# RustCrypto/elliptic-curves

Measured on AMD Instinct MI355X. Metric: k256 fixed-base scalar-muls/sec (variable-time: mul_by_generator_vartime), higher is better.
Workload: dtype u32 limbs (v_mad_u64_u32); 1 GPU; fixed_k256; curve=k256, units_per_gpu=1048576, units_total=1048576, window_bits=default, parallelism=shard1, input_sets=4, form=variable-time comb (ecgpu_batch_mul_base_dev = mul_by_generator_vartime)

## Files before the change

elliptic-curves_amd/csrc/ecgpu_batchinv.h:

```cpp
#pragma once

#include "ecgpu_point.h"
#include "ecgpu_scalar.h"

namespace ecgpu {

template <class R, class Load, class More, class Work>
ECGPU_HD void chain_walk(size_t first, size_t step, Load load, More has_next, Work work) {
    R cur, next;
    bool more = true;
    for (size_t j = first, it = 0;; j += step, it++) {
        if (more) load(j, next);
        if (it) work(j - step, cur);
        if (!more) break;
        cur = next;
        more = has_next(j);
    }
}

template <class P>
ECGPU_HD void batch_inv_lane(size_t t, size_t n, size_t nthreads, P& p) {
    using El = typename P::El;
    using Fwd = typename P::Fwd;
    using Back = typename P::Back;
    if (t >= n) return;
    El acc = p.one();
    chain_walk<Fwd>(t, nthreads, [&](size_t j, Fwd& r) { p.load_fwd(j, r); }, [&](size_t j) { return j + nthreads < n; },
                    [&](size_t j, const Fwd& r) {
                        El f;
                        const uint32_t cls = p.classify(j, r, f);
                        p.put_prefix(j, acc, cls);
                        if (cls == 0) acc = p.mul(acc, f);
                    });
    El inv = p.inv(acc);
    chain_walk<Back>(t + (n - 1 - t) / nthreads * nthreads, (size_t)0 - nthreads, [&](size_t j, Back& r) { p.load_back(j, r); },
                     [&](size_t j) { return j >= nthreads; },
                     [&](size_t j, const Back& r) {
                         El f, own;
                         const uint32_t cls = p.classify(j, r, f);
                         if (cls == 0) {
                             own = p.mul(p.prefix(j, r), inv);
                             inv = p.mul(inv, f);
                         }
                         p.emit(j, r, cls, own);
                     });
}

template <class Rec>
struct FieldLane : Rec {
    using F = typename Rec::F;
    using El = typename Rec::El;
    static constexpr int NL = Rec::NL, NS = Rec::NS;
    static_assert(NS > NL, "raw form has no spare word");
    ECGPU_HD El one() const { return F::one(); }
    ECGPU_HD El mul(const El& a, const El& b) const { return F::mul(a, b); }
    ECGPU_HD El inv(const El& a) const { return F::inv(a); }
    ECGPU_HD void put_prefix(size_t j, const El& acc, uint32_t cls) const {
        uint32_t w[NS];
#pragma unroll
        for (int i = 0; i < NS; i++) w[i] = i < NL ? acc.e.v[i] : 0u;
        w[NS - 1] = cls;
        this->io.put_prefix(j, w);
    }
    ECGPU_HD El prefix(size_t, const typename Rec::Back& r) const {
        Fe<NL> e;
#pragma unroll
        for (int i = 0; i < NL; i++) e.v[i] = r.pw[i];
        return F::template wrap<1, 1>(e);
    }
};

enum : int { NORM_WIRE = 0, NORM_PACKED = 1, NORM_COMPRESSED = 2 };
template <class C, int MODE, class Io>
struct NormRec {
    using F = Field<C>;
    using G = Group<C>;
    using El = typename F::M1;
    static constexpr int N = C::N, NL = C::NL, NS = F::NS;
    struct Fwd { Fe<NL> z; };
    struct Back { Proj<C> p; uint32_t pw[NS]; };
    Io& io;
    ECGPU_HD void load_fwd(size_t j, Fwd& r) const { r.z = io.load_z(j); }
    ECGPU_HD void load_back(size_t j, Back& r) const { r.p = io.load_point(j); io.get_prefix(j, r.pw); }
    ECGPU_HD uint32_t classify(size_t, const Fwd& r, El& f) const {
        f = G::m(r.z);
        return F::is_zero(f) ? 1u : 0u;
    }
    ECGPU_HD uint32_t classify(size_t, const Back& r, El& f) const {
        f = G::m(r.p.z);
        return r.pw[NS - 1];
    }
    ECGPU_HD void coord(uint32_t* w, const El& v) const {
        if constexpr (MODE == NORM_PACKED) F::pack(w, v);
        else F::to_canonical(w, v);
    }
    ECGPU_HD void emit(size_t j, const Back& r, uint32_t cls, const El& zinv) const {
        uint32_t w[N];
        if (cls) {
            if (MODE == NORM_PACKED) return;
#pragma unroll
            for (int i = 0; i < N; i++) w[i] = 0u;
            io.put_x(j, w);
            if (MODE == NORM_WIRE) io.put_y(j, w);
            io.put_flag(j, MODE == NORM_WIRE ? 1 : 0);
            return;
        }
        const El x = F::mul(G::m(r.p.x), zinv), y = F::mul(G::m(r.p.y), zinv);
        coord(w, x);
        io.put_x(j, w);
        coord(w, y);
        if (MODE != NORM_COMPRESSED) io.put_y(j, w);
        if (MODE != NORM_PACKED) io.put_flag(j, MODE == NORM_WIRE ? 0 : (uint8_t)(2u + (w[0] & 1u)));
    }
};
template <class C, int MODE, class Io>
ECGPU_HD void normalize_lane(size_t t, size_t n, size_t nthreads, Io& io) {
    FieldLane<NormRec<C, MODE, Io>> lane{{io}};
    batch_inv_lane(t, n, nthreads, lane);
}

template <class C, class Io>
struct ScalarInvLane {
    using S = ScalarN<C>;
    static constexpr int N = C::N;
    struct El { uint32_t v[N]; };
    struct Fwd {};
    struct Back {};
    Io& io;
    ECGPU_HD El one() const {
        El r = {{1u}};
        S::to_mont(r.v, r.v);
        return r;
    }
    ECGPU_HD El mul(const El& a, const El& b) const {
        El r;
        S::mont_mul(r.v, a.v, b.v);
        return r;
    }
    ECGPU_HD El inv(const El& acc) const {
        El x;
        S::inv(x.v, acc.v);
        S::to_mont(x.v, x.v);
        S::to_mont(x.v, x.v);
        return x;
    }
    ECGPU_HD void load_fwd(size_t, Fwd&) const {}
    ECGPU_HD void load_back(size_t, Back&) const {}
    template <class R>
    ECGPU_HD uint32_t classify(size_t j, const R&, El& f) const {
        uint32_t a[N];
        io.load(j, a);
        if (S::is_zero(a) || !S::in_range(a)) return 1u;
        S::to_mont(f.v, a);
        return 0u;
    }
    ECGPU_HD void put_prefix(size_t j, const El& acc, uint32_t) const { io.put_prefix(j, acc.v); }
    ECGPU_HD El prefix(size_t j, const Back&) const {
        El e;
        io.get_prefix(j, e.v);
        return e;
    }
    ECGPU_HD void emit(size_t j, const Back&, uint32_t cls, const El& ainv) const {
        El w = {};
        if (!cls) S::from_mont(w.v, ainv.v);
        io.put(j, w.v);
    }
};
template <class C, class Io>
ECGPU_HD void scalar_batch_inv_lane(size_t t, size_t n, size_t nthreads, Io& io) {
    ScalarInvLane<C, Io> lane{io};
    batch_inv_lane(t, n, nthreads, lane);
}

}
```

elliptic-curves_amd/csrc/ecgpu_field.h:

```cpp
#pragma once

#include "ecgpu_params.h"
#include "ecgpu_modinv.h"
#ifndef ECGPU_K256_ASM_REDUCE
#define ECGPU_K256_ASM_REDUCE 1
#endif
#if ECGPU_K256_ASM_REDUCE && defined(__HIP_DEVICE_COMPILE__) && (defined(__gfx950__) || defined(__gfx942__))
#define ECGPU_K256_ASM_REDUCE_ON 1
#include "ecgpu_k256_reduce_asm.h"
#else
#define ECGPU_K256_ASM_REDUCE_ON 0
#endif

namespace ecgpu {

template <class C, int L, int V>
struct Mag {
    Fe<C::NL> e;
};

static ECGPU_HD uint32_t opaque_const(uint32_t x) {
#if defined(__HIP_DEVICE_COMPILE__)
    asm("" : "+s"(x));
#endif
    return x;
}

template <class C>
struct Field {
    ECGPU_CONST int N = C::N;
    ECGPU_CONST int NL = C::NL;
    ECGPU_CONST int NS = (C::NL / 4 + 1) * 4;
    ECGPU_CONST int REPR = C::REPR;
    using E = Fe<C::NL>;
    using M1 = Mag<C, 1, 1>;

    ECGPU_CONST int MAXPROD = REPR == REPR_U29_K256 ? 7 : C::UC::MAXPROD;
    ECGPU_CONST int MAXMAG = REPR == REPR_U29_K256 ? 7 : C::UC::MAXMAG;

    using KC = consts::K256U;
    ECGPU_CONST uint32_t KMASK = (1u << 29) - 1;

    static ECGPU_HD void k_fold(uint64_t* lo, int j, uint64_t col) {
        uint32_t cl = (uint32_t)col, ch = (uint32_t)(col >> 32);
        lo[j] += (uint64_t)cl * KC::F0;
        lo[j + 1] += (uint64_t)cl * opaque_const(KC::F1);
        lo[j + 1] += (uint64_t)ch * KC::G1;
        lo[j + 2] += (uint64_t)ch * opaque_const(KC::G2);
    }
    static ECGPU_HD E k_reduce(uint64_t* c) {
#if ECGPU_K256_ASM_REDUCE_ON
        if constexpr (REPR == REPR_U29_K256) return k256_reduce_asm(c, KC::F0, KC::F1, KC::G1, KC::G2);
#endif
        return k_reduce_cpp(c);
    }
    static ECGPU_HD E k_reduce_cpp(uint64_t* c) {
        uint64_t lo[11];
#pragma unroll
        for (int k = 0; k < 9; k++) lo[k] = c[k];
        lo[9] = 0;
        lo[10] = 0;
#pragma unroll
        for (int k = 9; k < 16; k++) {
            const uint32_t cl = (uint32_t)c[k], ch = (uint32_t)(c[k] >> 32);
            c[k + 1] += (uint64_t)ch * opaque_const(8u);
            lo[k - 9] += (uint64_t)cl * KC::F0;
            lo[k - 8] += (uint64_t)cl * opaque_const(KC::F1);
        }
        k_fold(lo, 7, c[16]);
        {
            uint64_t c9 = lo[9], c10 = lo[10];
            const uint32_t cl = (uint32_t)c9, ch = (uint32_t)(c9 >> 32);
            c10 += (uint64_t)ch * opaque_const(8u);
            lo[0] += (uint64_t)cl * KC::F0;
            lo[1] += (uint64_t)cl * opaque_const(KC::F1);
            k_fold(lo, 1, c10);
        }
        E r;
        uint64_t v = lo[0];
#pragma unroll
        for (int k = 0; k < 8; k++) {
            r.v[k] = (uint32_t)v & KMASK;
            v = lo[k + 1] + (v >> 29);
        }
        r.v[8] = (uint32_t)v & KMASK;
        uint64_t top = v >> 29;
        uint32_t tl = (uint32_t)top, th = (uint32_t)(top >> 32);
        uint64_t t0 = (uint64_t)tl * KC::F0 + r.v[0];
        uint64_t t1 = (uint64_t)tl * opaque_const(KC::F1) + r.v[1];
        t1 += (uint64_t)th * KC::G1;
        uint64_t t2 = (uint64_t)th * opaque_const(KC::G2) + r.v[2];
        r.v[0] = (uint32_t)t0 & KMASK;
        t1 += t0 >> 29;
        r.v[1] = (uint32_t)t1 & KMASK;
        t2 += t1 >> 29;
        r.v[2] = (uint32_t)t2 & KMASK;
        r.v[3] += (uint32_t)(t2 >> 29);
        return r;
    }
    static ECGPU_HD void k_columns(uint64_t* c, const uint32_t* a, const uint32_t* b, bool accumulate) {
        if (!accumulate) {
#pragma unroll
            for (int k = 0; k < 17; k++) c[k] = 0;
        }
#pragma unroll
        for (int i = 0; i < 9; i++) {
#pragma unroll
            for (int j = 0; j < 9; j++) c[i + j] += (uint64_t)a[i] * b[j];
        }
    }
    static ECGPU_HD void k_columns_sqr(uint64_t* c, const uint32_t* a) {
        uint32_t a2[9];
#pragma unroll
        for (int k = 0; k < 17; k++) c[k] = 0;
#pragma unroll
        for (int j = 0; j < 9; j++) a2[j] = a[j] << 1;
#pragma unroll
        for (int i = 0; i < 9; i++) {
            c[2 * i] += (uint64_t)a[i] * a[i];
#pragma unroll
            for (int j = i + 1; j < 9; j++) c[i + j] += (uint64_t)a[i] * a2[j];
        }
    }
    static ECGPU_HD E k_norm(const E& a) {
        E r;
        uint32_t carry = 0;
#pragma unroll
        for (int k = 0; k < 9; k++) {
            uint32_t v = a.v[k] + carry;
            r.v[k] = v & KMASK;
            carry = v >> 29;
        }
        r.v[0] += carry * KC::F0;
        r.v[1] += carry * KC::F1;
        return r;
    }
    static ECGPU_HD E k_mul_small(const E& a, uint32_t k) {
        E r;
        uint64_t t = 0;
#pragma unroll
        for (int i = 0; i < 9; i++) {
            t += (uint64_t)a.v[i] * k;
            r.v[i] = (uint32_t)t & KMASK;
            t >>= 29;
        }
        uint32_t top = (uint32_t)t;
        uint64_t t0 = (uint64_t)top * KC::F0 + r.v[0];
        uint64_t t1 = (uint64_t)top * KC::F1 + r.v[1] + (t0 >> 29);
        r.v[0] = (uint32_t)t0 & KMASK;
        r.v[1] = (uint32_t)t1 & KMASK;
        r.v[2] += (uint32_t)(t1 >> 29);
        return r;
    }
    template <bool NORMED = false>
    static ECGPU_HD void k_to_words(uint32_t* w, const E& a) {
        E r;
        if constexpr (NORMED) r = a;
        else r = k_norm(k_norm(a));
#pragma unroll
        for (int rep = 0; rep < 2; rep++) {
            uint32_t carry = 0;
#pragma unroll
            for (int k = 0; k < 8; k++) {
                uint32_t v = r.v[k] + carry;
                r.v[k] = v & KMASK;
                carry = v >> 29;
            }
            uint32_t v8 = r.v[8] + carry;
            uint32_t e = v8 >> 24;
            r.v[8] = v8 & 0xFFFFFFu;
            r.v[0] += e * 977u;
            r.v[1] += e * 8u;
        }
        {
            uint32_t carry = 0;
#pragma unroll
            for (int k = 0; k < 8; k++) {
                uint32_t v = r.v[k] + carry;
                r.v[k] = v & KMASK;
                carry = v >> 29;
            }
            r.v[8] += carry;
        }
        E s = r;
        s.v[0] += 977u;
        s.v[1] += 8u;
        {
            uint32_t carry = 0;
#pragma unroll
            for (int k = 0; k < 8; k++) {
                uint32_t v = s.v[k] + carry;
                s.v[k] = v & KMASK;
                carry = v >> 29;
            }
            s.v[8] += carry;
        }
        bool ge = (s.v[8] >> 24) != 0;
        s.v[8] &= 0xFFFFFFu;
#pragma unroll
        for (int k = 0; k < 9; k++) r.v[k] = ge ? s.v[k] : r.v[k];
#pragma unroll
        for (int i = 0; i < 8; i++) {
            int bit = 32 * i, l = bit / 29, sh = bit % 29;
            uint64_t x = (uint64_t)r.v[l] >> sh;
            x |= (uint64_t)r.v[l + 1] << (29 - sh);
            if (l + 2 < 9) x |= (uint64_t)r.v[l + 2] << (58 - sh);
            w[i] = (uint32_t)x;
        }
    }
    template <int NLIMB, int BITS>
    static ECGPU_HD E words_to_limbs(const uint32_t* w) {
        E r;
#pragma unroll
        for (int l = 0; l < NLIMB; l++) {
            int bit = BITS * l, i = bit / 32, sh = bit % 32;
            uint64_t x = i < N ? (uint64_t)w[i] >> sh : 0;
            if (i + 1 < N) x |= (uint64_t)w[i + 1] << (32 - sh);
            r.v[l] = (uint32_t)x & ((1u << BITS) - 1);
        }
        return r;
    }

    using PC = typename C::UC;
    ECGPU_CONST int UN = PC::NL, UB = PC::B;
    ECGPU_CONST uint32_t PMASK = (1u << PC::B) - 1;

    static ECGPU_HD E p_reduce(uint64_t* c) {
        if constexpr (C::ID == CURVE_P256) {
#pragma unroll
            for (int i = 0; i < UN; i++) {
                uint32_t u = (uint32_t)c[i] & PMASK;
                c[i + 1] += (c[i] >> UB);
                c[i + 3] += (uint64_t)u * opaque_const(1u << 12);
                c[i + 6] += (uint64_t)u * opaque_const(1u << 24);
                c[i + 8] += (uint64_t)u * opaque_const(0xFFFFFFFFu);
            }
            E r;
            uint64_t v = c[UN];
#pragma unroll
            for (int k = 0; k < UN - 1; k++) {
                r.v[k] = (uint32_t)v & PMASK;
                v = c[UN + 1 + k] + (v >> UB);
            }
            r.v[UN - 1] = (uint32_t)v;
            return r;
        }
        if constexpr (C::ID == CURVE_P384) {
#pragma unroll
            for (int i = 0; i < UN; i++) {
                const int64_t ci = (int64_t)c[i];
                const int64_t u = (int64_t)((uint32_t)ci & PMASK);
                c[i + 1] = (uint64_t)((int64_t)c[i + 1] + (ci >> UB) + u * (int64_t)(int32_t)opaque_const(1u << 5));
                c[i + 3] = (uint64_t)((int64_t)c[i + 3] + u * (int64_t)(int32_t)opaque_const(0u - (1u << 15)));
                c[i + 4] = (uint64_t)((int64_t)c[i + 4] + u * (int64_t)(int32_t)opaque_const(0u - (1u << 20)));
                c[i + 14] = (uint64_t)((int64_t)c[i + 14] + u * (int64_t)(int32_t)opaque_const(1u << 6));
            }
            E r;
            int64_t v = (int64_t)c[UN];
#pragma unroll
            for (int k = 0; k < UN - 1; k++) {
                r.v[k] = (uint32_t)v & PMASK;
                v = (int64_t)c[UN + 1 + k] + (v >> UB);
            }
            r.v[UN - 1] = (uint32_t)v;
            return r;
        }
        if constexpr (C::ID == CURVE_P521) {
#pragma unroll
            for (int i = 0; i < UN; i++) {
                uint32_t u = (uint32_t)c[i] & PMASK;
                c[i + 1] += (c[i] >> UB);
                c[i + 19] += (uint64_t)u << 8;
            }
            E r;
            uint64_t v = c[UN];
#pragma unroll
            for (int k = 0; k < UN - 1; k++) {
                r.v[k] = (uint32_t)v & PMASK;
                v = c[UN + 1 + k] + (v >> UB);
            }
            r.v[UN - 1] = (uint32_t)v;
            return r;
        }
        if constexpr (C::ID == CURVE_SM2 || C::ID == CURVE_P224 || C::ID == CURVE_P192) {
            static_assert(HasBias<PC>::value, "sparse rows need the column biases");
#pragma unroll
            for (int i = 0; i < UN; i++) {
                uint32_t u;
                if constexpr (C::ID == CURVE_P224) {
                    u = (0u - (uint32_t)c[i]) & PMASK;
                    c[i + 1] += (c[i] + u) >> UB;
                } else {
                    u = (uint32_t)c[i] & PMASK;
                    c[i + 1] += c[i] >> UB;
                }
                const int64_t su = (int64_t)u;
                if constexpr (C::ID == CURVE_SM2) {
                    c[i + 2] += (uint64_t)u * opaque_const(1u << 8);
                    c[i + 3] = (uint64_t)((int64_t)c[i + 3] + su * (int64_t)(int32_t)opaque_const(0u - (1u << 12)));
                    c[i + 8] += (uint64_t)u * opaque_const(0xFFFFFFFFu);
                } else if constexpr (C::ID == CURVE_P224) {
                    c[i + 3] = (uint64_t)((int64_t)c[i + 3] + su * (int64_t)(int32_t)opaque_const(0u - (1u << 15)));
                    c[i + 8] += (uint64_t)u * opaque_const(1u << 8);
                } else {
                    c[i + 2] = (uint64_t)((int64_t)c[i + 2] + su * (int64_t)(int32_t)opaque_const(0u - (1u << 12)));
                    c[i + 7] += (uint64_t)u * opaque_const(1u << 10);
                }
            }
            E r;
            uint64_t v = c[UN];
#pragma unroll
            for (int k = 0; k < UN - 1; k++) {
                r.v[k] = (uint32_t)v & PMASK;
                v = c[UN + 1 + k] + (v >> UB);
            }
            r.v[UN - 1] = (uint32_t)v;
            return r;
        }
        if constexpr (C::ID == CURVE_BIGN256) {
            static_assert(UB == 28 && UN == 10, "bign256: 10 x 28 limbs");
#pragma unroll
            for (int i = 0; i < UN; i++) {
                const int64_t ci = (int64_t)c[i];
                const int64_t u = (int64_t)(((uint32_t)ci * PC::PINV) & PMASK);
                const int64_t t = ci + u * (int64_t)(int32_t)opaque_const(0u - 189u);
                c[i + 1] = (uint64_t)((int64_t)c[i + 1] + (t >> UB));
                c[i + 9] = (uint64_t)((int64_t)c[i + 9] + u * (int64_t)(int32_t)opaque_const(16u));
            }
            E r;
            int64_t v = (int64_t)c[UN];
#pragma unroll
            for (int k = 0; k < UN - 1; k++) {
                r.v[k] = (uint32_t)v & PMASK;
                v = (int64_t)c[UN + 1 + k] + (v >> UB);
            }
            r.v[UN - 1] = (uint32_t)v;
            return r;
        }
        if constexpr (!PC::P0_IS_MINUS_ONE && !PC::P0_IS_ONE) {
#pragma unroll
            for (int i = 0; i < UN; i++) {
                uint32_t u = ((uint32_t)c[i] * PC::PINV) & PMASK;
#pragma unroll
                for (int j = 0; j < UN; j++) {
                    if (PC::P[j] != 0) c[i + j] += (uint64_t)u * opaque_const(PC::P[j]);
                }
                c[i + 1] += c[i] >> UB;
            }
            E r;
            uint64_t v = c[UN];
#pragma unroll
            for (int k = 0; k < UN - 1; k++) {
                r.v[k] = (uint32_t)v & PMASK;
                v = c[UN + 1 + k] + (v >> UB);
            }
            r.v[UN - 1] = (uint32_t)v;
            return r;
        }
        if constexpr (PC::P0_IS_ONE) {
            static_assert(PC::P[0] == 1, "p0 = 1 expected");
#pragma unroll
            for (int i = 0; i < UN; i++) {
                uint32_t u = (0u - (uint32_t)c[i]) & PMASK;
                c[i + 1] += (c[i] + u) >> UB;
#pragma unroll
                for (int j = 1; j < UN; j++) {
                    if (PC::P[j] != 0) c[i + j] += (uint64_t)u * opaque_const(PC::P[j]);
                }
            }
            E r;
            uint64_t v = c[UN];
#pragma unroll
            for (int k = 0; k < UN - 1; k++) {
                r.v[k] = (uint32_t)v & PMASK;
                v = c[UN + 1 + k] + (v >> UB);
            }
            r.v[UN - 1] = (uint32_t)v;
            return r;
        }
#pragma unroll
        for (int i = 0; i < UN; i++) {
            uint32_t u = (uint32_t)c[i] & PMASK;
            c[i + 1] += (c[i] >> UB);
            c[i + 1] += (uint64_t)u * opaque_const(PC::P[1] + 1u);
#pragma unroll
            for (int j = 2; j < UN; j++) {
                if (PC::P[j] != 0) c[i + j] += (uint64_t)u * opaque_const(PC::P[j]);
            }
        }
        E r;
        uint64_t v = c[UN];
#pragma unroll
        for (int k = 0; k < UN - 1; k++) {
            r.v[k] = (uint32_t)v & PMASK;
            v = c[UN + 1 + k] + (v >> UB);
        }
        r.v[UN - 1] = (uint32_t)v;
        return r;
    }
    template <class T, class = void>
    struct HasBias : std::false_type {};
    template <class T>
    struct HasBias<T, std::void_t<decltype(T::SPARSE_BIAS)>> : std::true_type {};
    static ECGPU_HD void p_columns_init(uint64_t* c) {
#pragma unroll
        for (int k = 0; k < 2 * UN + 1; k++) {
            if constexpr (HasBias<PC>::value) c[k] = PC::BIAS[k];
            else c[k] = 0;
        }
    }
    static ECGPU_HD void p_columns(uint64_t* c, const uint32_t* a, const uint32_t* b, bool accumulate) {
        if (!accumulate) p_columns_init(c);
#pragma unroll
        for (int i = 0; i < UN; i++) {
#pragma unroll
            for (int j = 0; j < UN; j++) c[i + j] += (uint64_t)a[i] * b[j];
        }
    }
    static ECGPU_HD void p_columns_sqr(uint64_t* c, const uint32_t* a) {
        uint32_t a2[UN];
        p_columns_init(c);
#pragma unroll
        for (int j = 0; j < UN; j++) a2[j] = a[j] << 1;
#pragma unroll
        for (int i = 0; i < UN; i++) {
            c[2 * i] += (uint64_t)a[i] * a[i];
#pragma unroll
            for (int j = i + 1; j < UN; j++) c[i + j] += (uint64_t)a[i] * a2[j];
        }
    }
    static ECGPU_HD E p_norm(const E& a) {
        E r;
        uint32_t carry = 0;
#pragma unroll
        for (int k = 0; k < UN - 1; k++) {
            uint32_t v = a.v[k] + carry;
            r.v[k] = v & PMASK;
            carry = v >> UB;
        }
        r.v[UN - 1] = a.v[UN - 1] + carry;
        return r;
    }
    static ECGPU_HD E p_cond_sub(const E& a) {
        E d;
        int32_t borrow = 0;
#pragma unroll
        for (int k = 0; k < UN - 1; k++) {
            int32_t t = (int32_t)a.v[k] - (int32_t)PC::P[k] + borrow;
            d.v[k] = (uint32_t)t & PMASK;
            borrow = t >> UB;
        }
        int32_t tt = (int32_t)a.v[UN - 1] - (int32_t)PC::P[UN - 1] + borrow;
        d.v[UN - 1] = (uint32_t)tt;
        bool lt = tt < 0;
        E r;
#pragma unroll
        for (int k = 0; k < UN; k++) r.v[k] = lt ? a.v[k] : d.v[k];
        return r;
    }
    static ECGPU_HD void p_limbs_to_words(uint32_t* w, const E& r) {
#pragma unroll
        for (int i = 0; i < N; i++) {
            int bit = 32 * i, l = bit / UB, sh = bit % UB;
            uint64_t x = (uint64_t)r.v[l] >> sh;
            if (l + 1 < UN) x |= (uint64_t)r.v[l + 1] << (UB - sh);
            if (l + 2 < UN) x |= (uint64_t)r.v[l + 2] << (2 * UB - sh);
            w[i] = (uint32_t)x;
        }
    }
    static ECGPU_HD E p_const(const uint32_t* limbs) {
        E r;
#pragma unroll
        for (int k = 0; k < UN; k++) r.v[k] = limbs[k];
        return r;
    }
    static ECGPU_HD E p_mont_mul(const E& a, const E& b) {
        uint64_t c[2 * UN + 1];
        p_columns(c, a.v, b.v, false);
        return p_reduce(c);
    }

    template <int L, int V>
    static ECGPU_HD void check_mag(const E& e) {
#if defined(ECGPU_BOUNDS_CHECK) && !defined(__HIP_DEVICE_COMPILE__)
        if constexpr (REPR == REPR_U29_K256) {
            for (int i = 0; i < NL; i++)
                if ((uint64_t)e.v[i] > (uint64_t)L * KC::LB) { __builtin_trap(); }
        } else if constexpr (REPR == REPR_U28_MONT) {
            for (int i = 0; i < NL - 1; i++)
                if ((uint64_t)e.v[i] > (uint64_t)L * PC::LB) { __builtin_trap(); }
            if ((uint64_t)e.v[NL - 1] > (uint64_t)V * PC::TOP1 + PC::TOP1 / 2) { __builtin_trap(); }
        }
#else
        (void)e;
#endif
    }
    template <int L, int V>
    static ECGPU_HD Mag<C, L, V> wrap(const E& e) {
        check_mag<L, V>(e);
        Mag<C, L, V> r;
        r.e = e;
        return r;
    }
    static ECGPU_HD M1 zero() {
        M1 r;
#pragma unroll
        for (int i = 0; i < NL; i++) r.e.v[i] = 0;
        return r;
    }
    static ECGPU_HD M1 one() {
        M1 r = zero();
        if constexpr (REPR == REPR_U28_MONT) {
            r.e = p_const(PC::ONE);
        } else {
            r.e.v[0] = 1;
        }
        return r;
    }

    template <int LA, int VA, int LB, int VB>
    static ECGPU_HD auto add(const Mag<C, LA, VA>& a, const Mag<C, LB, VB>& b) {
        static_assert(LA + LB <= MAXMAG, "limb magnitude overflow in add: normalise an operand first");
        Mag<C, LA + LB, VA + VB> r;
#pragma unroll
        for (int i = 0; i < NL; i++) r.e.v[i] = a.e.v[i] + b.e.v[i];
        check_mag<LA + LB, VA + VB>(r.e);
        return r;
    }
    template <int LA, int VA>
    static ECGPU_HD auto dbl(const Mag<C, LA, VA>& a) { return add(a, a); }

    template <int LA, int VA, int LB, int VB>
    static ECGPU_HD auto sel(bool flag, const Mag<C, LA, VA>& a, const Mag<C, LB, VB>& b) {
        Mag<C, (LA > LB ? LA : LB), (VA > VB ? VA : VB)> r;
#pragma unroll
        for (int i = 0; i < NL; i++) r.e.v[i] = flag ? a.e.v[i] : b.e.v[i];
        return r;
    }

    template <int LB, int VB>
    static ECGPU_HD auto neg(const Mag<C, LB, VB>& b) {
        if constexpr (REPR == REPR_U29_K256) {
            constexpr int m = LB > VB ? LB : VB;
            static_assert(m <= KC::ZMAX, "no subtraction constant for this magnitude: normalise first");
            Mag<C, m + 1, m + 1> r;
            check_mag<LB, VB>(b.e);
#pragma unroll
            for (int i = 0; i < NL; i++) r.e.v[i] = KC::Z[m][i] - b.e.v[i];
            check_mag<m + 1, m + 1>(r.e);
            return r;
        } else {
            static_assert(LB <= PC::LMAX && VB <= PC::VMAX, "no subtraction constant for this magnitude");
            Mag<C, LB + 1, VB + 1> r;
            check_mag<LB, VB>(b.e);
#pragma unroll
            for (int i = 0; i < NL; i++) r.e.v[i] = PC::Z[LB][VB][i] - b.e.v[i];
            check_mag<LB + 1, VB + 1>(r.e);
            return r;
        }
    }
    template <int LA, int VA, int LB, int VB>
    static ECGPU_HD auto sub(const Mag<C, LA, VA>& a, const Mag<C, LB, VB>& b) {
        return add(a, neg(b));
    }

    template <int LA, int VA, int LB, int VB>
    static ECGPU_HD M1 mul(const Mag<C, LA, VA>& a, const Mag<C, LB, VB>& b) {
        if constexpr (REPR == REPR_U29_K256) {
            static_assert(LA * LB <= MAXPROD, "k256 mul: limb magnitude product too large");
            uint64_t c[17];
            k_columns(c, a.e.v, b.e.v, false);
            return wrap<1, 1>(k_reduce(c));
        } else {
            static_assert(LA * LB <= MAXPROD, "p256 mul: limb magnitude product too large");
            static_assert((long)VA * VB <= (1L << PC::VLIMIT_LOG2), "mul: value magnitude product too large");
            uint64_t c[2 * UN + 1];
            p_columns(c, a.e.v, b.e.v, false);
            return wrap<1, 1>(p_reduce(c));
        }
    }
    template <int LA, int VA>
    static ECGPU_HD M1 sqr(const Mag<C, LA, VA>& a) {
        if constexpr (REPR == REPR_U29_K256) {
            static_assert(LA * LA <= MAXPROD, "k256 sqr: limb magnitude too large");
            uint64_t c[17];
            k_columns_sqr(c, a.e.v);
            return wrap<1, 1>(k_reduce(c));
        } else {
            static_assert(LA * LA <= MAXPROD, "p256 sqr: limb magnitude too large");
            uint64_t c[2 * UN + 1];
            p_columns_sqr(c, a.e.v);
            return wrap<1, 1>(p_reduce(c));
        }
    }
    template <int LA, int VA, int LB, int VB, int LC, int VC, int LD, int VD>
    static ECGPU_HD M1 mul2(const Mag<C, LA, VA>& a, const Mag<C, LB, VB>& b, const Mag<C, LC, VC>& c,
                            const Mag<C, LD, VD>& d) {
        if constexpr (REPR == REPR_U29_K256) {
            static_assert(LA * LB + LC * LD <= MAXPROD, "k256 mul2: limb magnitude products too large");
            uint64_t col[17];
            k_columns(col, a.e.v, b.e.v, false);
            k_columns(col, c.e.v, d.e.v, true);
            return wrap<1, 1>(k_reduce(col));
        } else {
            static_assert(LA * LB + LC * LD <= MAXPROD, "p256 mul2: limb magnitude products too large");
            static_assert((long)VA * VB + (long)VC * VD <= (1L << PC::VLIMIT_LOG2), "mul2: value magnitudes too large");
            uint64_t col[2 * UN + 1];
            p_columns(col, a.e.v, b.e.v, false);
            p_columns(col, c.e.v, d.e.v, true);
            return wrap<1, 1>(p_reduce(col));
        }
    }
    template <int LC, int VC>
    static ECGPU_HD void k_columns_sub(uint64_t* col, const Mag<C, LC, VC>& c) {
        constexpr int m = LC > VC ? LC : VC;
        static_assert(m <= KC::ZMAX, "no subtraction constant for this magnitude: normalise first");
        check_mag<LC, VC>(c.e);
        const uint32_t one = opaque_const(1u);
#pragma unroll
        for (int k = 0; k < 9; k++) col[k] += (uint64_t)(KC::Z[m][k] - c.e.v[k]) * one;
    }
    template <int LC, int VC>
    static ECGPU_HD void p_columns_sub(uint64_t* col, const Mag<C, LC, VC>& c) {
        static_assert(LC <= PC::LMAX && VC <= PC::VMAX, "no subtraction constant for this magnitude");
        check_mag<LC, VC>(c.e);
        const uint32_t one = opaque_const(1u);
#pragma unroll
        for (int k = 0; k < UN; k++) col[UN + k] += (uint64_t)(PC::Z[LC][VC][k] - c.e.v[k]) * one;
    }
    template <int LA, int VA, int LB, int VB, int LC, int VC>
    static ECGPU_HD auto mul_sub(const Mag<C, LA, VA>& a, const Mag<C, LB, VB>& b, const Mag<C, LC, VC>& c) {
        if constexpr (REPR == REPR_U29_K256) {
            static_assert(LA * LB <= MAXPROD, "k256 mul_sub: limb magnitude product too large");
            uint64_t col[17];
            k_columns(col, a.e.v, b.e.v, false);
            k_columns_sub(col, c);
            return wrap<1, 1>(k_reduce(col));
        } else {
            static_assert(LA * LB <= MAXPROD, "mul_sub: limb magnitude product too large");
            static_assert((long)VA * VB <= (1L << PC::VLIMIT_LOG2), "mul_sub: value magnitude product too large");
            uint64_t col[2 * UN + 1];
            p_columns(col, a.e.v, b.e.v, false);
            p_columns_sub(col, c);
            return wrap<1, VC + 2>(p_reduce(col));
        }
    }
    template <int LA, int VA, int LC, int VC>
    static ECGPU_HD auto sqr_sub(const Mag<C, LA, VA>& a, const Mag<C, LC, VC>& c) {
        if constexpr (REPR == REPR_U29_K256) {
            static_assert(LA * LA <= MAXPROD, "k256 sqr_sub: limb magnitude too large");
            uint64_t col[17];
            k_columns_sqr(col, a.e.v);
            k_columns_sub(col, c);
            return wrap<1, 1>(k_reduce(col));
        } else {
            static_assert(LA * LA <= MAXPROD, "sqr_sub: limb magnitude too large");
            static_assert((long)VA * VA <= (1L << PC::VLIMIT_LOG2), "sqr_sub: value magnitude too large");
            uint64_t col[2 * UN + 1];
            p_columns_sqr(col, a.e.v);
            p_columns_sub(col, c);
            return wrap<1, VC + 2>(p_reduce(col));
        }
    }
    template <int LA, int VA>
    static ECGPU_HD auto norm(const Mag<C, LA, VA>& a) {
        if constexpr (REPR == REPR_U29_K256) return wrap<1, 1>(k_norm(a.e));
        else return wrap<1, VA>(p_norm(a.e));
    }
    ECGPU_CONST int SQLIM = MAXPROD >= 49 ? 7 : (MAXPROD >= 16 ? 4 : (MAXPROD >= 4 ? 2 : 1));
    template <int LIM, int LA, int VA>
    static ECGPU_HD auto fit(const Mag<C, LA, VA>& a) {
        if constexpr (LA > LIM) return norm(a);
        else return a;
    }
    template <uint32_t K, int LA, int VA>
    static ECGPU_HD M1 mul_small(const Mag<C, LA, VA>& a) {
        static_assert(REPR == REPR_U29_K256, "mul_small is only provided for k256");
        static_assert(K < (1u << 12), "constant too large");
        return wrap<1, 1>(k_mul_small(a.e, K));
    }

    static ECGPU_HD M1 from_canonical(const uint32_t* w) {
        if constexpr (REPR == REPR_U29_K256) {
            return wrap<1, 1>(words_to_limbs<9, 29>(w));
        } else {
            E a = words_to_limbs<UN, UB>(w);
            return wrap<1, 1>(p_mont_mul(a, p_const(PC::R2)));
        }
    }
    template <int LA, int VA>
    static ECGPU_HD void to_canonical(uint32_t* w, const Mag<C, LA, VA>& a) {
        if constexpr (REPR == REPR_U29_K256) {
            check_mag<LA, VA>(a.e);
            k_to_words<(LA <= 1)>(w, a.e);
        } else {
            static_assert(LA <= MAXPROD, "normalise before to_canonical");
            E onep;
#pragma unroll
            for (int k = 0; k < UN; k++) onep.v[k] = k == 0 ? 1u : 0u;
            E r = p_cond_sub(p_mont_mul(a.e, onep));
            p_limbs_to_words(w, r);
        }
    }
    template <int LA, int VA>
    static ECGPU_HD void pack(uint32_t* w, const Mag<C, LA, VA>& a) {
        if constexpr (REPR == REPR_U29_K256) {
            check_mag<LA, VA>(a.e);
            k_to_words<(LA <= 1)>(w, a.e);
        } else {
            static_assert(LA <= MAXPROD, "normalise before pack");
            E r = p_cond_sub(p_mont_mul(a.e, p_const(PC::ONE)));
            p_limbs_to_words(w, r);
        }
    }
    static ECGPU_HD M1 unpack(const uint32_t* w) {
        if constexpr (REPR == REPR_U29_K256) {
            return wrap<1, 1>(words_to_limbs<9, 29>(w));
        } else {
            return wrap<1, 1>(words_to_limbs<UN, UB>(w));
        }
    }

    template <int LA, int VA>
    static ECGPU_HD bool is_zero(const Mag<C, LA, VA>& a) {
        uint32_t w[N];
        pack(w, a);
        return mp_is_zero<N>(w);
    }
    template <int LA, int VA, int LB, int VB>
    static ECGPU_HD bool eq(const Mag<C, LA, VA>& a, const Mag<C, LB, VB>& b) {
        return is_zero(norm(sub(a, b)));
    }

    static ECGPU_HD M1 from_bytes(const uint8_t* be, bool* ok) {
        uint32_t w[N];
        load_be_wire<C>(w, be);
        *ok = !mp_geq<N>(w, C::P);
        return from_canonical(w);
    }
    template <int LA, int VA>
    static ECGPU_HD void to_bytes(uint8_t* be, const Mag<C, LA, VA>& a) {
        uint32_t w[N];
        to_canonical(w, a);
        store_be_wire<C>(be, w);
    }

    static ECGPU_HD M1 sqr_n(M1 x, int n) {
#pragma unroll 1
        for (int i = 0; i < n; i++) x = sqr(x);
        return x;
    }
    template <bool VAR = false>
    static ECGPU_HD M1 inv(const M1& a) {
        uint32_t w[N], r[N];
        pack(w, a);
        if constexpr (VAR) ModInv<N>::invert_var(r, w, C::P);
        else ModInv<N>::invert(r, w, C::P);
        M1 x = unpack(r);
        if constexpr (REPR == REPR_U28_MONT) {
            M1 r2 = wrap<1, 1>(p_const(PC::R2));
            x = mul(mul(x, r2), r2);
        }
        return x;
    }
    static ECGPU_HD M1 inv_fermat(const M1& a) {
        if constexpr (REPR == REPR_U29_K256) {
            M1 x2 = mul(sqr(a), a);
            M1 x3 = mul(sqr(x2), a);
            M1 x6 = mul(sqr_n(x3, 3), x3);
            M1 x9 = mul(sqr_n(x6, 3), x3);
            M1 x11 = mul(sqr_n(x9, 2), x2);
            M1 x22 = mul(sqr_n(x11, 11), x11);
            M1 x44 = mul(sqr_n(x22, 22), x22);
            M1 x88 = mul(sqr_n(x44, 44), x44);
            M1 x176 = mul(sqr_n(x88, 88), x88);
            M1 x220 = mul(sqr_n(x176, 44), x44);
            M1 x223 = mul(sqr_n(x220, 3), x3);
            M1 t = mul(sqr_n(x223, 23), x22);
            t = mul(sqr_n(t, 5), a);
            t = mul(sqr_n(t, 3), x2);
            t = mul(sqr_n(t, 2), a);
            return t;
        } else if constexpr (REPR == REPR_U28_MONT && C::ID == CURVE_P256) {
            M1 x2 = mul(sqr(a), a);
            M1 x3 = mul(sqr(x2), a);
            M1 x6 = mul(sqr_n(x3, 3), x3);
            M1 x12 = mul(sqr_n(x6, 6), x6);
            M1 x15 = mul(sqr_n(x12, 3), x3);
            M1 x30 = mul(sqr_n(x15, 15), x15);
            M1 x32 = mul(sqr_n(x30, 2), x2);
            M1 t = mul(sqr_n(x32, 32), a);
            t = mul(sqr_n(t, 128), x32);
            t = mul(sqr_n(t, 32), x32);
            t = mul(sqr_n(t, 30), x30);
            t = mul(sqr_n(t, 2), a);
            return t;
        } else {
            M1 tab[16];
            tab[0] = one();
            tab[1] = a;
#pragma unroll 1
            for (int i = 2; i < 16; i++) tab[i] = mul(tab[i - 1], a);
            uint32_t e[N];
#pragma unroll
            for (int i = 0; i < N; i++) e[i] = C::P[i];
            {
                uint32_t borrow = 2;
#pragma unroll
                for (int i = 0; i < N; i++) {
                    const uint32_t v = e[i];
                    e[i] = v - borrow;
                    borrow = v < borrow ? 1u : 0u;
                }
            }
            M1 r = one();
#pragma unroll 1
            for (int i = 8 * N - 1; i >= 0; i--) {
                uint32_t nib = (e[i >> 3] >> ((i & 7) * 4)) & 0xF;
                r = sqr(sqr(sqr(sqr(r))));
                if (nib) r = mul(r, tab[nib]);
            }
            return r;
        }
    }
    static ECGPU_HD M1 sqrt_sylow(const M1& a, bool* ok) {
        static_assert(C::ID == CURVE_P224, "Tonelli-Shanks constants exist for p224 only");
        constexpr int S = C::UC::SYLOW_S;
        M1 x2 = mul(sqr(a), a);
        M1 x3 = mul(sqr(x2), a);
        M1 x6 = mul(sqr_n(x3, 3), x3);
        M1 x12 = mul(sqr_n(x6, 6), x6);
        M1 x24 = mul(sqr_n(x12, 12), x12);
        M1 x48 = mul(sqr_n(x24, 24), x24);
        M1 x96 = mul(sqr_n(x48, 48), x48);
        M1 x120 = mul(sqr_n(x96, 24), x24);
        M1 x126 = mul(sqr_n(x120, 6), x6);
        M1 w = mul(sqr(x126), a);
        M1 r = mul(w, a);
        M1 t = mul(r, w);
        M1 gpow = wrap<1, 1>(p_const(C::UC::SYLOW_GINV));
        M1 ghalf = one();
#pragma unroll 1
        for (int i = 0; i < S; i++) {
            const M1 u = sqr_n(t, S - 1 - i);
            const bool bit = !eq(u, one());
            const M1 tg = mul(t, gpow), rg = mul(r, ghalf);
            t = wrap<1, 1>(sel(bit, tg, t).e);
            r = wrap<1, 1>(sel(bit && i > 0, rg, r).e);
            ghalf = gpow;
            gpow = sqr(gpow);
        }
        *ok = eq(sqr(r), a);
        return r;
    }
    static ECGPU_HD M1 sqrt(const M1& a, bool* ok) {
        M1 r;
        if constexpr (C::ID == CURVE_P224) {
            return sqrt_sylow(a, ok);
        } else if constexpr (REPR == REPR_U29_K256) {
            M1 x2 = mul(sqr(a), a);
            M1 x3 = mul(sqr(x2), a);
            M1 x6 = mul(sqr_n(x3, 3), x3);
            M1 x9 = mul(sqr_n(x6, 3), x3);
            M1 x11 = mul(sqr_n(x9, 2), x2);
            M1 x22 = mul(sqr_n(x11, 11), x11);
            M1 x44 = mul(sqr_n(x22, 22), x22);
            M1 x88 = mul(sqr_n(x44, 44), x44);
            M1 x176 = mul(sqr_n(x88, 88), x88);
            M1 x220 = mul(sqr_n(x176, 44), x44);
            M1 x223 = mul(sqr_n(x220, 3), x3);
            r = mul(sqr_n(x223, 23), x22);
            r = mul(sqr_n(r, 6), x2);
            r = sqr_n(r, 2);
        } else if constexpr (REPR == REPR_U28_MONT && C::ID == CURVE_P256) {
            M1 t11 = mul(a, sqr(a));
            M1 t1111 = mul(t11, sqr_n(t11, 2));
            M1 t8 = mul(t1111, sqr_n(t1111, 4));
            M1 x16 = mul(sqr_n(t8, 8), t8);
            r = mul(sqr_n(x16, 16), x16);
            r = mul(sqr_n(r, 32), a);
            r = mul(sqr_n(r, 96), a);
            r = sqr_n(r, 94);
        } else if constexpr (C::ID == CURVE_P521) {
            r = sqr_n(a, 519);
        } else {
            M1 tab[16];
            tab[0] = one();
            tab[1] = a;
#pragma unroll 1
            for (int i = 2; i < 16; i++) tab[i] = mul(tab[i - 1], a);
            uint32_t e[N];
            {
                uint64_t c = 1;
#pragma unroll
                for (int i = 0; i < N; i++) {
                    c += C::P[i];
                    e[i] = (uint32_t)c;
                    c >>= 32;
                }
#pragma unroll
                for (int i = 0; i < N; i++) e[i] = (e[i] >> 2) | (i + 1 < N ? e[i + 1] << 30 : 0u);
            }
            r = one();
#pragma unroll 1
            for (int i = 8 * N - 1; i >= 0; i--) {
                uint32_t nib = (e[i >> 3] >> ((i & 7) * 4)) & 0xF;
                r = sqr(sqr(sqr(sqr(r))));
                if (nib) r = mul(r, tab[nib]);
            }
        }
        *ok = eq(sqr(r), a);
        return r;
    }
};

}
```

elliptic-curves_amd/csrc/ecgpu_fixedmul.h:

```cpp
#pragma once

#include "ecgpu_point.h"
#include "ecgpu_recode.h"

namespace ecgpu {

template <class C, class Table>
ECGPU_HD Affine<C> load_entry(const Table& table, int window, uint32_t index) {
    PackedPoint<2 * C::N> pw;
    table.load(pw, window, index);
    Affine<C> q;
    q.x = Field<C>::unpack(pw.w).e;
    q.y = Field<C>::unpack(pw.w + C::N).e;
    return q;
}

template <class C>
constexpr bool COMB_NEEDS_CHECK = C::ORDER[C::N - 1] < 0xF0000000u;

template <class C, class Table>
ECGPU_HD Proj<C> fixed_base_mul(const uint32_t* k_in, const Table& table, int w, int nwin, const Fe<C::NL>& b) {
    using G = Group<C>;
    constexpr int N = C::N;
    uint32_t k[N];
#pragma unroll
    for (int i = 0; i < N; i++) k[i] = k_in[i];
    const bool flip = fold_scalar<N>(k, C::ORDER);
    uint32_t carry = 0;
    int state = 0;
    Xyzz<C> acc;
    acc.x = acc.y = acc.zz = acc.zzz = Field<C>::one().e;
#pragma unroll 1
    for (int j = 0; j < nwin; j++) {
        int d = signed_window_step(get_bits<N>(k, j * w, w), w, &carry);
        if (d != 0) {
            Affine<C> q = load_entry<C>(table, j, (uint32_t)(d < 0 ? -d : d) - 1);
            const bool neg = (d < 0) != flip;
            if (state == 2) {
                acc = G::xyzz_madd(acc, q, neg);
            } else if (state == 1) {
                Affine<C> a;
                a.x = acc.x;
                a.y = acc.y;
                acc = G::xyzz_mmadd(a, q, neg);
                state = 2;
            } else {
                if (neg) q.y = G::neg_coord(q.y);
                acc.x = q.x;
                acc.y = q.y;
                state = 1;
            }
        }
    }
    if (state == 0) return G::identity();
    if (state == 1) {
        Affine<C> a;
        a.x = acc.x;
        a.y = acc.y;
        return G::from_affine(a);
    }
    if constexpr (COMB_NEEDS_CHECK<C>) {
        if (Field<C>::is_zero(G::mj(acc.zz))) {
            uint32_t carry2 = 0;
            Proj<C> r = G::identity();
#pragma unroll 1
            for (int j = 0; j < nwin; j++) {
                int d = signed_window_step(get_bits<N>(k, j * w, w), w, &carry2);
                if (d != 0) {
                    Affine<C> q = load_entry<C>(table, j, (uint32_t)(d < 0 ? -d : d) - 1);
                    r = G::add_mixed(r, q, b, (d < 0) != flip);
                }
            }
            return r;
        }
    }
    return G::xyzz_to_proj(acc);
}


}
```

elliptic-curves_amd/csrc/ecgpu_selftest_point_raw.h:

```cpp
#pragma once

#include "ecgpu_point.h"
#include "ecgpu_ctmul.h"

namespace ecgpu {

ECGPU_CONST int SELFTEST_POINT_RAW_MAX_STEPS = 64;

template <class C>
ECGPU_HD bool selftest_point_raw(int op, const uint32_t* p, const uint32_t* q, uint32_t* r) {
    using G = Group<C>;
    constexpr int NL = C::NL;
    const int code = op & 0xFF, steps = op >> 8;
    Fe<NL> a[4], b[4], o[4];
#pragma unroll
    for (int k = 0; k < 4; k++)
#pragma unroll
        for (int t = 0; t < NL; t++) {
            a[k].v[t] = p[k * NL + t];
            b[k].v[t] = q[k * NL + t];
            o[k].v[t] = 0;
        }
    const Fe<NL> cb = G::curve_b();
    Proj<C> P, Q;
    P.x = a[0]; P.y = a[1]; P.z = a[2];
    Q.x = b[0]; Q.y = b[1]; Q.z = b[2];
    Jac<C> J;
    J.x = a[0]; J.y = a[1]; J.z = a[2];
    Xyzz<C> S;
    S.x = a[0]; S.y = a[1]; S.zz = a[2]; S.zzz = a[3];
    Affine<C> pa, qa;
    pa.x = a[0]; pa.y = a[1];
    qa.x = b[0]; qa.y = b[1];
    auto put_p = [&](const Proj<C>& v) { o[0] = v.x; o[1] = v.y; o[2] = v.z; };
    auto put_j = [&](const Jac<C>& v) { o[0] = v.x; o[1] = v.y; o[2] = v.z; };
    auto put_s = [&](const Xyzz<C>& v) { o[0] = v.x; o[1] = v.y; o[2] = v.zz; o[3] = v.zzz; };
    bool known = steps == 0 || ((code == 15 || code == 16) && steps <= SELFTEST_POINT_RAW_MAX_STEPS);
    if (known) {
        switch (code) {
        case 0: put_p(G::add(P, Q, cb)); break;
        case 1: put_p(G::add(P, Q, cb, true)); break;
        case 2: put_p(G::add_mixed(P, qa, cb)); break;
        case 3: put_p(G::add_mixed(P, qa, cb, true)); break;
        case 4: put_p(G::dbl(P, cb)); break;
        case 5: put_p(G::neg(P)); break;
        case 6: put_p(ct_dbl4<C>(P, cb)); break;
        case 7: put_j(G::jac_dbl(J)); break;
        case 8: put_j(G::jac_madd(J, qa, false)); break;
        case 9: put_j(G::jac_madd(J, qa, true)); break;
        case 10: put_p(G::jac_to_proj(J)); break;
        case 11: put_s(G::xyzz_madd(S, qa, false)); break;
        case 12: put_s(G::xyzz_madd(S, qa, true)); break;
        case 13: put_s(G::xyzz_mmadd(pa, qa, false)); break;
        case 14: put_p(G::xyzz_to_proj(S)); break;
        case 15:
#pragma unroll 1
            for (int s = 0; s < steps; s++) P = G::dbl(G::add(P, Q, cb), cb);
            put_p(P);
            break;
        case 16:
#pragma unroll 1
            for (int s = 0; s < steps; s++) {
#pragma unroll 1
                for (int d = 0; d < 4; d++) J = G::jac_dbl(J);
                J = G::jac_madd(J, qa, false);
            }
            put_j(J);
            break;
        case 17: o[0].v[0] = G::is_identity(P) ? 1u : 0u; break;
        default: known = false;
        }
    }
#pragma unroll
    for (int k = 0; k < 4; k++)
#pragma unroll
        for (int t = 0; t < NL; t++) r[k * NL + t] = o[k].v[t];
    return known;
}

}
```

Measured before the change: 1.822 billion scalar-muls/s.

## Add wave-uniform fast path for k256 comb walk and cheaper zero test

For curves without the comb check and with 8 scalar words, the fixed-base comb loop now pulls digits by shifting a local scalar copy with alignbit, replacing get_bits. While every lane in the wave has a nonzero digit it runs a branch-free xyzz_madd loop that skips the per-lane state dispatch. It falls back to the generic state-based loop once any lane sees a zero digit. A cheaper k256-specific is_zero_short replaces pack-based zero detection in batch normalization, and a selftest case checks it against the existing is_zero.

```diff
diff --git a/elliptic-curves_amd/csrc/ecgpu_batchinv.h b/elliptic-curves_amd/csrc/ecgpu_batchinv.h
--- a/elliptic-curves_amd/csrc/ecgpu_batchinv.h
+++ b/elliptic-curves_amd/csrc/ecgpu_batchinv.h
@@ -84,7 +84,7 @@
     ECGPU_HD void load_back(size_t j, Back& r) const { r.p = io.load_point(j); io.get_prefix(j, r.pw); }
     ECGPU_HD uint32_t classify(size_t, const Fwd& r, El& f) const {
         f = G::m(r.z);
-        return F::is_zero(f) ? 1u : 0u;
+        return F::is_zero_short(f) ? 1u : 0u;
     }
     ECGPU_HD uint32_t classify(size_t, const Back& r, El& f) const {
         f = G::m(r.p.z);
diff --git a/elliptic-curves_amd/csrc/ecgpu_field.h b/elliptic-curves_amd/csrc/ecgpu_field.h
--- a/elliptic-curves_amd/csrc/ecgpu_field.h
+++ b/elliptic-curves_amd/csrc/ecgpu_field.h
@@ -151,6 +151,37 @@
         r.v[1] = (uint32_t)t1 & KMASK;
         r.v[2] += (uint32_t)(t1 >> 29);
         return r;
+    }
+    template <bool NORMED = false>
+    static ECGPU_HD bool k_is_zero(const E& a) {
+        E r;
+        if constexpr (NORMED) r = a;
+        else r = k_norm(k_norm(a));
+        uint32_t carry = 0;
+#pragma unroll
+        for (int k = 0; k < 8; k++) {
+            uint32_t v = r.v[k] + carry;
+            r.v[k] = v & KMASK;
+            carry = v >> 29;
+        }
+        const uint32_t v8 = r.v[8] + carry, e = v8 >> 24;
+        r.v[8] = v8 & 0xFFFFFFu;
+        r.v[0] += e * 977u;
+        r.v[1] += e * 8u;
+        carry = 0;
+#pragma unroll
+        for (int k = 0; k < 8; k++) {
+            uint32_t v = r.v[k] + carry;
+            r.v[k] = v & KMASK;
+            carry = v >> 29;
+        }
+        r.v[8] += carry;
+        uint32_t any = r.v[0], notp = (r.v[0] ^ 0x1FFFFC2Fu) | (r.v[1] ^ 0x1FFFFFF7u) | (r.v[8] ^ 0xFFFFFFu);
+#pragma unroll
+        for (int k = 1; k < 9; k++) any |= r.v[k];
+#pragma unroll
+        for (int k = 2; k < 8; k++) notp |= r.v[k] ^ KMASK;
+        return any == 0 || notp == 0;
     }
     template <bool NORMED = false>
     static ECGPU_HD void k_to_words(uint32_t* w, const E& a) {
@@ -726,6 +757,15 @@
         uint32_t w[N];
         pack(w, a);
         return mp_is_zero<N>(w);
+    }
+    template <int LA, int VA>
+    static ECGPU_HD bool is_zero_short(const Mag<C, LA, VA>& a) {
+        if constexpr (REPR == REPR_U29_K256) {
+            check_mag<LA, VA>(a.e);
+            return k_is_zero<(LA <= 1)>(a.e);
+        } else {
+            return is_zero(a);
+        }
     }
     template <int LA, int VA, int LB, int VB>
     static ECGPU_HD bool eq(const Mag<C, LA, VA>& a, const Mag<C, LB, VB>& b) {
diff --git a/elliptic-curves_amd/csrc/ecgpu_fixedmul.h b/elliptic-curves_amd/csrc/ecgpu_fixedmul.h
--- a/elliptic-curves_amd/csrc/ecgpu_fixedmul.h
+++ b/elliptic-curves_amd/csrc/ecgpu_fixedmul.h
@@ -18,6 +18,53 @@
 template <class C>
 constexpr bool COMB_NEEDS_CHECK = C::ORDER[C::N - 1] < 0xF0000000u;
 
+template <int N>
+ECGPU_HD uint32_t take_low_bits(uint32_t* k, int w) {
+    const uint32_t raw = k[0] & ((1u << w) - 1);
+#pragma unroll
+    for (int i = 0; i + 1 < N; i++) {
+#if defined(__HIP_DEVICE_COMPILE__)
+        k[i] = __builtin_amdgcn_alignbit(k[i + 1], k[i], (uint32_t)w);
+#else
+        k[i] = (uint32_t)((((uint64_t)k[i + 1] << 32) | k[i]) >> w);
+#endif
+    }
+    k[N - 1] >>= w;
+    return raw;
+}
+
+ECGPU_HD bool wave_all(bool pred) {
+#if defined(__HIP_DEVICE_COMPILE__)
+    return __builtin_amdgcn_ballot_w64(!pred) == 0;
+#else
+    return pred;
+#endif
+}
+
+template <class C>
+constexpr bool COMB_FAST_WALK = !COMB_NEEDS_CHECK<C> && C::N == 8;
+
+template <class C, class Table>
+ECGPU_HD void comb_add(int& state, Xyzz<C>& acc, const Table& table, int j, int d, bool flip) {
+    using G = Group<C>;
+    Affine<C> q = load_entry<C>(table, j, (uint32_t)(d < 0 ? -d : d) - 1);
+    const bool neg = (d < 0) != flip;
+    if (state == 2) {
+        acc = G::xyzz_madd(acc, q, neg);
+    } else if (state == 1) {
+        Affine<C> a;
+        a.x = acc.x;
+        a.y = acc.y;
+        acc = G::xyzz_mmadd(a, q, neg);
+        state = 2;
+    } else {
+        if (neg) q.y = G::neg_coord(q.y);
+        acc.x = q.x;
+        acc.y = q.y;
+        state = 1;
+    }
+}
+
 template <class C, class Table>
 ECGPU_HD Proj<C> fixed_base_mul(const uint32_t* k_in, const Table& table, int w, int nwin, const Fe<C::NL>& b) {
     using G = Group<C>;
@@ -30,26 +77,41 @@
     int state = 0;
     Xyzz<C> acc;
     acc.x = acc.y = acc.zz = acc.zzz = Field<C>::one().e;
+    if constexpr (!COMB_FAST_WALK<C>) {
 #pragma unroll 1
-    for (int j = 0; j < nwin; j++) {
-        int d = signed_window_step(get_bits<N>(k, j * w, w), w, &carry);
-        if (d != 0) {
-            Affine<C> q = load_entry<C>(table, j, (uint32_t)(d < 0 ? -d : d) - 1);
-            const bool neg = (d < 0) != flip;
-            if (state == 2) {
-                acc = G::xyzz_madd(acc, q, neg);
-            } else if (state == 1) {
-                Affine<C> a;
-                a.x = acc.x;
-                a.y = acc.y;
-                acc = G::xyzz_mmadd(a, q, neg);
-                state = 2;
-            } else {
-                if (neg) q.y = G::neg_coord(q.y);
-                acc.x = q.x;
-                acc.y = q.y;
-                state = 1;
+        for (int j = 0; j < nwin; j++) {
+            int d = signed_window_step(get_bits<N>(k, j * w, w), w, &carry);
+            if (d != 0) comb_add<C>(state, acc, table, j, d, flip);
+        }
+    } else {
+        uint32_t ks[N];
+#pragma unroll
+        for (int i = 0; i < N; i++) ks[i] = k[i];
+        int j = 0;
+        int d = signed_window_step(take_low_bits<N>(ks, w), w, &carry);
+        if (wave_all(d != 0)) {
+            comb_add<C>(state, acc, table, 0, d, flip);
+            j = 1;
+            if (nwin > 1) {
+                d = signed_window_step(take_low_bits<N>(ks, w), w, &carry);
+                if (wave_all(d != 0)) {
+                    comb_add<C>(state, acc, table, 1, d, flip);
+                    j = 2;
+#pragma unroll 1
+                    while (j < nwin) {
+                        d = signed_window_step(take_low_bits<N>(ks, w), w, &carry);
+                        if (!wave_all(d != 0)) break;
+                        Affine<C> q = load_entry<C>(table, j, (uint32_t)(d < 0 ? -d : d) - 1);
+                        acc = G::xyzz_madd(acc, q, (d < 0) != flip);
+                        j++;
+                    }
+                }
             }
+        }
+#pragma unroll 1
+        while (j < nwin) {
+            if (d != 0) comb_add<C>(state, acc, table, j, d, flip);
+            if (++j < nwin) d = signed_window_step(take_low_bits<N>(ks, w), w, &carry);
         }
     }
     if (state == 0) return G::identity();
diff --git a/elliptic-curves_amd/csrc/ecgpu_selftest_point_raw.h b/elliptic-curves_amd/csrc/ecgpu_selftest_point_raw.h
--- a/elliptic-curves_amd/csrc/ecgpu_selftest_point_raw.h
+++ b/elliptic-curves_amd/csrc/ecgpu_selftest_point_raw.h
@@ -68,6 +68,10 @@
             put_j(J);
             break;
         case 17: o[0].v[0] = G::is_identity(P) ? 1u : 0u; break;
+        case 19:
+            o[0].v[0] = Field<C>::is_zero_short(G::m(P.z)) ? 1u : 0u;
+            o[0].v[1] = Field<C>::is_zero(G::m(P.z)) ? 1u : 0u;
+            break;
         default: known = false;
         }
     }
```

Result: faster. 1.846 billion scalar-muls/s, median of 6 (+1.3%).
